# davidkelley/searchlite

Hardware: NVIDIA B200
Metric: bm25_top10_queries_per_sec (higher is better)
Workload: dtype f32

## Files before the change

### searchlite_b200/csrc/slg_engine.cu

```cuda
#include "slg_host.h"

#include <cub/cub.cuh>
#include <fcntl.h>
#include <sys/mman.h>
#include <sys/stat.h>
#include <unistd.h>

#include "slg_filter.cuh"
#include "slg_phrase.cuh"
#include "slg_postimage.cuh"
#include "slg_residency.cuh"
#include "slg_segfiles.h"

using namespace slg;

namespace slg {
std::string &open_error() {
  thread_local std::string e;
  return e;
}
cudaStream_t &pool_stream() {
  thread_local cudaStream_t s = nullptr;
  return s;
}
// ... 87 lines not shown
  d.col_stride = 0;
  d.term_ub = nullptr;
  d.term_bits = nullptr;
  d.pres_bits = nullptr;
  d.bits_stride = 0;
  d.n_terms = s->n_terms;
  d.doc_count = s->doc_count;
  d.k1p1 = s->k1 + 1.0f;
  d.min_nk = host_nk(s->min_doc_len, s->avgdl, s->k1, s->b);
  d.term_field = n_fields > 1 ? s->term_field.as<uint8_t>() : nullptr;
  for (uint32_t f = 0; f < kMaxFields; f++)
    d.min_nk_f[f] = f < n_fields ? host_nk(s->f_min_len[f], s->f_avgdl[f], s->k1, s->b) : d.min_nk;

  if (ix->resident_scores && s->n_blocks) {
    SLG_CUDA(ix, s->post_score.alloc(s->n_post_padded * 4));
    SLG_CUDA(ix, cudaMemsetAsync(s->post_score.p, 0, s->n_post_padded * 4, st));
    SLG_CUDA(ix, s->mb_max.alloc((s->n_post_padded / 32 + 1) * 4));
    SLG_CUDA(ix, cudaMemsetAsync(s->mb_max.p, 0, (s->n_post_padded / 32 + 1) * 4, st));
    slg_score_postings_kernel<<<s->n_blocks, 128, 0, st>>>(d, s->n_blocks, s->post_score.as<float>(), s->mb_max.as<float>());
    count_launch(ix);
    SLG_CUDA(ix, cudaGetLastError());
    d.post_score = s->post_score.as<float>();
    d.mb_max = s->mb_max.as<float>();
    if (ix->dense_den && s->doc_count) {
      const uint64_t stride = align_up((uint64_t)s->doc_count, 4096) + 4096;
      std::vector<uint32_t> cand;
      for (uint64_t t = 0; t < s->n_terms; t++) {
        const uint64_t df = s->h_df[t];
        if (df >= ix->dense_min_df && df * ix->dense_den >= s->doc_count) cand.push_back((uint32_t)t);
      }
      std::sort(cand.begin(), cand.end(), [&](uint32_t a, uint32_t b2) { return s->h_df[a] != s->h_df[b2] ? s->h_df[a] > s->h_df[b2] : a < b2; });
      const uint64_t max_cols = std::min<uint64_t>(65535, ix->max_column_bytes / (stride * 4));
      if (cand.size() > max_cols) cand.resize(max_cols);
      if (!cand.empty()) {
        std::vector<int32_t> tcol(s->n_terms, -1);
        for (size_t c = 0; c < cand.size(); c++) tcol[cand[c]] = (int32_t)c;
        DevBuf d_terms;
        SLG_CUDA(ix, d_terms.alloc(cand.size() * 4));
        SLG_CUDA(ix, cudaMemcpyAsync(d_terms.p, cand.data(), cand.size() * 4, cudaMemcpyHostToDevice, st));
        SLG_CUDA(ix, s->term_col.alloc(s->n_terms * 4));
        SLG_CUDA(ix, cudaMemcpyAsync(s->term_col.p, tcol.data(), s->n_terms * 4, cudaMemcpyHostToDevice, st));
        SLG_CUDA(ix, s->cols.alloc(cand.size() * stride * 4));
        SLG_CUDA(ix, cudaMemsetAsync(s->cols.p, 0, cand.size() * stride * 4, st));
        s->n_cols = (uint32_t)cand.size();
        s->col_stride = stride;
        d.col_stride = stride;
        for (size_t c0 = 0; c0 < cand.size(); c0 += 32768) {
          const uint32_t nc = (uint32_t)std::min<size_t>(32768, cand.size() - c0);
          slg_fill_columns_kernel<<<dim3(256, nc), 256, 0, st>>>(d, d_terms.as<uint32_t>() + c0, nc,
                                                                  s->cols.as<float>() + c0 * stride);
          count_launch(ix);
        }
        SLG_CUDA(ix, cudaGetLastError());
        s->tmax_stride = (uint32_t)(stride / 512);
        SLG_CUDA(ix, s->col_tmax.alloc(cand.size() * s->tmax_stride * 4));
        {
          const uint64_t warps = (uint64_t)cand.size() * s->tmax_stride;
          slg_column_tmax_kernel<<<(unsigned)((warps * 32 + 255) / 256), 256, 0, st>>>(s->cols.as<float>(), stride, (uint32_t)cand.size(),
                                                                                     s->tmax_stride, s->col_tmax.as<float>());
          count_launch(ix);
        }
        SLG_CUDA(ix, cudaGetLastError());
        SLG_CUDA(ix, cudaStreamSynchronize(st));
        s->h_term_col = std::move(tcol);
        d.cols = s->cols.as<float>();
        d.term_col = s->term_col.as<int32_t>();
        d.col_tmax = s->col_tmax.as<float>();
        d.tmax_stride = s->tmax_stride;
      }
    }
  }
  if (d.post_score && s->n_terms) {
    SLG_CUDA(ix, s->term_ub.alloc(s->n_terms * 4));
    SLG_CUDA(ix, cudaMemsetAsync(s->term_ub.p, 0, s->n_terms * 4, st));
    ScanDev sc{};
    sc.ut_term = nullptr;
    sc.ut_max = s->term_ub.as<float>();
    slg_term_max_kernel<<<dim3((unsigned)((s->n_terms + 7) / 8), kMaxSlices), 256, 0, st>>>(d, sc, (uint32_t)s->n_terms);
    count_launch(ix);
    SLG_CUDA(ix, cudaGetLastError());
    d.term_ub = s->term_ub.as<float>();
  }
  if (ix->resident_scores && ix->bitmap_den && s->doc_count && s->n_blocks) {
    const uint32_t stride = (uint32_t)align_up(((uint64_t)s->doc_count + 31) / 32, 32);
    std::vector<uint32_t> cand;
    for (uint64_t t = 0; t < s->n_terms; t++) {
      const uint64_t df = s->h_df[t];
      if (df >= 64 && df * ix->bitmap_den >= s->doc_count && (s->h_term_col.empty() || s->h_term_col[t] < 0)) cand.push_back((uint32_t)t);
    }
    std::sort(cand.begin(), cand.end(), [&](uint32_t a, uint32_t b2) { return s->h_df[a] != s->h_df[b2] ? s->h_df[a] > s->h_df[b2] : a < b2; });
    const uint64_t max_rows = std::min<uint64_t>(32768, ix->max_bitmap_bytes / ((uint64_t)stride * 4));
    if (cand.size() > max_rows) cand.resize(max_rows);
    if (!cand.empty()) {
      std::vector<int32_t> tb(s->n_terms, -1);
      for (size_t r = 0; r < cand.size(); r++) tb[cand[r]] = (int32_t)r;
      DevBuf d_terms;
      SLG_CUDA(ix, d_terms.alloc(cand.size() * 4));
      SLG_CUDA(ix, cudaMemcpyAsync(d_terms.p, cand.data(), cand.size() * 4, cudaMemcpyHostToDevice, st));
      SLG_CUDA(ix, s->term_bits.alloc(s->n_terms * 4));
      SLG_CUDA(ix, cudaMemcpyAsync(s->term_bits.p, tb.data(), s->n_terms * 4, cudaMemcpyHostToDevice, st));
      SLG_CUDA(ix, s->pres_bits.alloc(cand.size() * (uint64_t)stride * 4));
      SLG_CUDA(ix, cudaMemsetAsync(s->pres_bits.p, 0, cand.size() * (uint64_t)stride * 4, st));
      slg_fill_presence_kernel<<<dim3(64, (unsigned)cand.size()), 256, 0, st>>>(d, d_terms.as<uint32_t>(), (uint32_t)cand.size(), s->pres_bits.as<uint32_t>(), stride);
      count_launch(ix);
      SLG_CUDA(ix, cudaGetLastError());
      SLG_CUDA(ix, cudaStreamSynchronize(st));
      s->n_bitmaps = (uint32_t)cand.size();
      d.term_bits = s->term_bits.as<int32_t>();
      d.pres_bits = s->pres_bits.as<uint32_t>();
      d.bits_stride = stride;
    }
  }
  ix->ctr.resident_bytes += s->resident();
  for (auto &old : ix->segs)
    if (old->ord == s->ord) {
      ix->ctr.resident_bytes -= old->resident();
      old = std::move(seg);
      return SLG_OK;
    }
  ix->segs.push_back(std::move(seg));
  std::sort(ix->segs.begin(), ix->segs.end(), [](const auto &a, const auto &b2) { return a->ord < b2->ord; });
  return SLG_OK;
}

int32_t build_layout(slg_index *ix, Segment *s) {
  cudaStream_t st = ix->stream;
  std::vector<uint64_t> start(s->n_terms + 1);
  std::vector<uint32_t> blk(s->n_terms + 1);
  uint64_t pos = 0, nb = 0, np = 0;
  for (uint64_t t = 0; t < s->n_terms; t++) {
    start[t] = pos;
    blk[t] = (uint32_t)nb;
    uint32_t df = s->h_df[t];
    np += df;
    pos += align_up(df, kTermAlign);
    nb += (df + kBlock - 1) / kBlock;
    if (nb > 0xFFFFFFF0ull) return fail(ix, SLG_ERR_UNSUPPORTED, "segment has too many posting blocks");
  }
  start[s->n_terms] = pos;
  blk[s->n_terms] = (uint32_t)nb;
  s->n_postings = np;
  s->n_post_padded = pos + 1024;
  s->n_blocks = (uint32_t)nb;
  SLG_CUDA(ix, s->term_start.alloc((s->n_terms + 1) * 8));
  SLG_CUDA(ix, s->term_blk.alloc((s->n_terms + 1) * 4));
  SLG_CUDA(ix, s->term_df.alloc(std::max<uint64_t>(s->n_terms, 1) * 4));
  SLG_CUDA(ix, cudaMemcpyAsync(s->term_start.p, start.data(), (s->n_terms + 1) * 8, cudaMemcpyHostToDevice, st));
  SLG_CUDA(ix, cudaMemcpyAsync(s->term_blk.p, blk.data(), (s->n_terms + 1) * 4, cudaMemcpyHostToDevice, st));
  if (s->n_terms) SLG_CUDA(ix, cudaMemcpyAsync(s->term_df.p, s->h_df.data(), s->n_terms * 4, cudaMemcpyHostToDevice, st));
  SLG_CUDA(ix, s->post_doc.alloc(s->n_post_padded * 4));
  SLG_CUDA(ix, s->post_tf.alloc(s->n_post_padded));
  SLG_CUDA(ix, cudaMemsetAsync(s->post_doc.p, 0xFF, s->n_post_padded * 4, st));
  SLG_CUDA(ix, cudaMemsetAsync(s->post_tf.p, 0, s->n_post_padded, st));
  SLG_CUDA(ix, s->blk_max_doc.alloc((size_t)std::max(s->n_blocks, 1u) * 4));
  SLG_CUDA(ix, s->blk_max_tf.alloc((size_t)std::max(s->n_blocks, 1u) * 4));
  SLG_CUDA(ix, s->term_max_tf.alloc(std::max<uint64_t>(s->n_terms, 1) * 4));
  SLG_CUDA(ix, s->term_wide.alloc(std::max<uint64_t>(s->n_terms, 1) * 8));
  SLG_CUDA(ix, cudaMemsetAsync(s->term_wide.p, 0xFF, std::max<uint64_t>(s->n_terms, 1) * 8, st));
  SLG_CUDA(ix, cudaStreamSynchronize(st));
  s->h_start = std::move(start);
  return SLG_OK;
}

int32_t build_wide(slg_index *ix, Segment *s, const uint64_t *d_csr_off, const uint32_t *d_csr_tfs, const uint4 *d_ovf = nullptr,
                   uint32_t n_ovf = 0) {
  cudaStream_t st = ix->stream;
  if (!s->n_terms) return SLG_OK;
  if (s->n_blocks) {
    DevBuf bad;
    SLG_CUDA(ix, bad.alloc(4));
    SLG_CUDA(ix, cudaMemsetAsync(bad.p, 0, 4, st));
    slg_validate_postings_kernel<<<s->n_blocks, 128, 0, st>>>(s->term_start.as<uint64_t>(), s->term_blk.as<uint32_t>(), s->term_df.as<uint32_t>(),
                                                              s->n_terms, s->n_blocks, s->post_doc.as<uint32_t>(), s->doc_count, bad.as<uint32_t>());
    count_launch(ix);
    uint32_t n_bad = 0;
    SLG_CUDA(ix, cudaMemcpyAsync(&n_bad, bad.p, 4, cudaMemcpyDeviceToHost, st));
    SLG_CUDA(ix, cudaStreamSynchronize(st));
    if (n_bad)
      return fail(ix, SLG_ERR_INVALID, "segment %u: %u postings name a doc outside the segment's %u docs or break the ascending order of their list",
                  s->ord, n_bad, s->doc_count);
  }
  slg_term_max_tf_kernel<<<(unsigned)((s->n_terms + 255) / 256), 256, 0, st>>>(s->term_blk.as<uint32_t>(), s->blk_max_tf.as<float>(),
                                                                              s->n_terms, s->term_max_tf.as<float>());
  count_launch(ix);
  std::vector<float> mtf(s->n_terms);
  SLG_CUDA(ix, cudaMemcpyAsync(mtf.data(), s->term_max_tf.p, s->n_terms * 4, cudaMemcpyDeviceToHost, st));
  SLG_CUDA(ix, cudaStreamSynchronize(st));
  std::vector<uint32_t> wide_terms;
  std::vector<uint64_t> wide_off;
// ... 1421 lines not shown
```

### searchlite_b200/csrc/slg_residency.cuh

```cuda
#pragma once
#include "slg_kernels.cuh"

namespace slg {

static __global__ void __launch_bounds__(256) slg_plan_walk_kernel(SegmentDev seg, const uint32_t *ut_term, const uint32_t *row_u,
                                                              uint32_t n_rows, uint32_t tile_docs, uint32_t n_tiles,
                                                              bool column_rows, uint32_t *rng) {
  const uint32_t r = blockIdx.x;
  if (r >= n_rows) return;
  const uint32_t term = ut_term[row_u ? row_u[r] : r];
  uint32_t *out = rng + (uint64_t)r * (n_tiles + 1);
  const uint32_t step = gridDim.y * blockDim.x;
  const uint32_t first = blockIdx.y * blockDim.x + threadIdx.x;
  if (term >= seg.n_terms) {
    for (uint32_t j = first; j <= n_tiles; j += step) out[j] = 0u;
    return;
  }
  if (!column_rows && seg.term_col && seg.term_col[term] >= 0) return;
  const uint32_t df = seg.term_df[term];
  const uint32_t *d = seg.post_doc + seg.term_start[term];
  if ((uint64_t)df <= 8ull * (n_tiles + 1)) {
    for (uint32_t i = first; i <= df; i += step) {
      const uint32_t a = i ? d[i - 1] / tile_docs + 1 : 0u;
      const uint32_t b = i < df ? d[i] / tile_docs : n_tiles;
      for (uint32_t j = a; j <= b; j++) out[j] = i;
    }
  } else {
    for (uint32_t j = first; j <= n_tiles; j += step) {
      const uint64_t target = (uint64_t)j * tile_docs;
      uint32_t lo = 0, hi = df;
      while (lo < hi) {
        const uint32_t mid = (lo + hi) >> 1;
        if (d[mid] < target) lo = mid + 1;
        else hi = mid;
      }
      out[j] = lo;
    }
  }
}

static __global__ void __launch_bounds__(128) slg_score_postings_kernel(SegmentDev seg, uint32_t n_blocks, float *post_score, float *mb_max) {
  const uint32_t blk = blockIdx.x;
  if (blk >= n_blocks) return;
  __shared__ uint32_t s_term;
  if (threadIdx.x == 0) {
    uint64_t lo = 0, hi = seg.n_terms;
    while (lo + 1 < hi) {
      const uint64_t mid = (lo + hi) >> 1;
      if (seg.term_blk[mid] <= blk) lo = mid;
      else hi = mid;
    }
    s_term = (uint32_t)lo;
  }
  __syncthreads();
  const uint32_t term = s_term;
  const uint32_t i = (blk - seg.term_blk[term]) * kBlock + threadIdx.x;
  const uint32_t df = seg.term_df[term];
  const uint64_t base = seg.term_start[term];
  float s = 0.0f;
  if (i < df) {
    const uint32_t doc = seg.post_doc[base + i];
    uint32_t tf = seg.post_tf[base + i];
    const uint64_t wide = seg.term_wide[term];
    if (tf == 255u && wide != ~0ull) tf = seg.tf_wide[wide + i];
    s = bm25_contrib_fast(tf, seg.term_idf[term], seg.k1p1, seg_nk(seg, term)[doc], 1.0f);
    post_score[base + i] = s;
  }
  float m = s;
  for (int o = 16; o > 0; o >>= 1) m = fmaxf(m, __shfl_xor_sync(0xFFFFFFFFu, m, o));
  const uint32_t i0 = (blk - seg.term_blk[term]) * kBlock + (threadIdx.x & ~31u);
  if ((threadIdx.x & 31) == 0 && i0 < ((df + 31u) & ~31u)) mb_max[(base + i0) >> 5] = m;
}

static __global__ void slg_fill_columns_kernel(SegmentDev seg, const uint32_t *col_terms, uint32_t n_cols, float *cols) {
  const uint32_t c = blockIdx.y;
  if (c >= n_cols) return;
  const uint32_t term = col_terms[c];
  const uint32_t df = seg.term_df[term];
  const uint64_t base = seg.term_start[term];
  float *col = cols + (uint64_t)c * seg.col_stride;
  for (uint32_t i = blockIdx.x * blockDim.x + threadIdx.x; i < df; i += gridDim.x * blockDim.x)
    col[seg.post_doc[base + i]] = seg.post_score[base + i];
}

static __global__ void slg_fill_presence_kernel(SegmentDev seg, const uint32_t *bm_terms, uint32_t n_rows, uint32_t *bits, uint32_t stride) {
  const uint32_t r = blockIdx.y;
  if (r >= n_rows) return;
  const uint32_t term = bm_terms[r];
  const uint32_t df = seg.term_df[term];
  const uint32_t *d = seg.post_doc + seg.term_start[term];
  uint32_t *row = bits + (uint64_t)r * stride;
  for (uint32_t i = blockIdx.x * blockDim.x + threadIdx.x; i < df; i += gridDim.x * blockDim.x) {
    const uint32_t doc = d[i];
    atomicOr(row + (doc >> 5), 1u << (doc & 31));
  }
}

static __global__ void slg_column_tmax_kernel(const float *cols, uint64_t col_stride, uint32_t n_cols, uint32_t tmax_stride, float *tmax) {
  const uint64_t w = ((uint64_t)blockIdx.x * blockDim.x + threadIdx.x) >> 5;
  const int lane = threadIdx.x & 31;
  if (w >= (uint64_t)n_cols * tmax_stride) return;
  const uint32_t c = (uint32_t)(w / tmax_stride), j = (uint32_t)(w % tmax_stride);
  const float4 *p = reinterpret_cast<const float4 *>(cols + (uint64_t)c * col_stride + (uint64_t)j * 512) + lane;
  float m = 0.0f;
#pragma unroll
  for (int i = 0; i < 4; i++) {
    const float4 v = p[i * 32];
    m = fmaxf(m, fmaxf(fmaxf(v.x, v.y), fmaxf(v.z, v.w)));
  }
  for (int o = 16; o > 0; o >>= 1) m = fmaxf(m, __shfl_xor_sync(0xFFFFFFFFu, m, o));
  if (lane == 0) tmax[w] = m;
}

}
```

### searchlite_b200/csrc/slg_scan_kernel.cuh

```cuda
#pragma once
#include "slg_stream_kernel.cuh"

namespace slg {

constexpr uint32_t kScanChunk = 4096;
constexpr int kScanWarps = 8;
constexpr uint32_t kScanQueue = 512;

struct __align__(16) ScanPair {
  uint64_t base;
  uint32_t df;
  uint32_t qslot_t;
  uint32_t qi;
  float w;
  float others;
  float ne_prefix;
  int32_t filter;
  uint32_t first_item;
  uint32_t pad[2];
};

struct ScanDev {
  const uint32_t *ut_term;
  float *ut_max;
// ... 205 lines not shown

static __global__ void __launch_bounds__(1024) slg_scan_order_kernel(WarpBatchDev wb, ScanDev sc) {
  __shared__ uint32_t s_hist[33], s_cur[33], s_carry;
  const uint32_t tid = threadIdx.x, nthr = blockDim.x;
  const uint32_t n = wb.n_queries * kWarpMaxTerms;
  if (tid < 33) s_hist[tid] = 0u;
  __syncthreads();
  for (uint32_t i = tid; i < n; i += nthr) {
    const uint32_t df = sc.pairs[i].df;
    if (df) atomicAdd(&s_hist[32 - __clz(df)], 1u);
  }
  __syncthreads();
  if (tid == 0) {
    uint32_t run = 0;
    for (int b = 0; b < 33; b++) {
      s_cur[b] = run;
      run += s_hist[b];
    }
    *sc.n_pairs = run;
    s_carry = 0;
  }
  __syncthreads();
  for (uint32_t i = tid; i < n; i += nthr) {
    const uint32_t df = sc.pairs[i].df;
    if (df) sc.order[atomicAdd(&s_cur[32 - __clz(df)], 1u)] = i;
  }
  __syncthreads();
  const uint32_t np = *sc.n_pairs;
  __shared__ uint32_t s_scan[1024];
  for (uint32_t b0 = 0; b0 < np; b0 += nthr) {
    const uint32_t i = b0 + tid;
    uint32_t c = 0;
    if (i < np) c = (sc.pairs[sc.order[i]].df + sc.chunk - 1) / sc.chunk;
    s_scan[tid] = c;
    __syncthreads();
    for (uint32_t o = 1; o < nthr; o <<= 1) {
      const uint32_t v = tid >= o ? s_scan[tid - o] : 0u;
      __syncthreads();
      s_scan[tid] += v;
      __syncthreads();
    }
    const uint32_t excl = s_scan[tid] - c + s_carry;
    if (i < np) {
      sc.item_start[i] = excl;
      sc.pairs[sc.order[i]].first_item = excl;
    }
    __syncthreads();
    if (tid == nthr - 1) s_carry += s_scan[tid];
    __syncthreads();
  }
  if (tid == 0) {
    sc.item_start[np] = s_carry;
    *sc.n_items = min(s_carry, sc.items_cap);
  }
}

static __global__ void __launch_bounds__(256) slg_scan_items_kernel(ScanDev sc) {
  const uint32_t i = blockIdx.x * blockDim.x + threadIdx.x;
  const uint32_t n_items = *sc.n_items, np = *sc.n_pairs;
  if (i >= n_items) return;
  uint32_t lo = 0, hi = np;
  while (lo + 1 < hi) {
    const uint32_t mid = (lo + hi) >> 1;
    if (sc.item_start[mid] <= i) lo = mid;
    else hi = mid;
  }
  sc.items[i] = lo;
}

template <bool PRUNE, bool POOLS, bool MUST>
__global__ void __launch_bounds__(kScanWarps * 32, 4) slg_scan_kernel(SegmentDev seg, WarpBatchDev wb, ScanDev sc) {
  __shared__ __align__(16) unsigned long long s_cand[kScanWarps][kWarpCand];
  __shared__ uint32_t s_hist[kScanWarps][POOLS ? 256 : 1];
  __shared__ uint32_t s_qidx[kScanWarps][kScanQueue];
  __shared__ float s_qval[kScanWarps][kScanQueue];
  const int lane = threadIdx.x & 31, warp = threadIdx.x >> 5;
  unsigned long long *cand = s_cand[warp];
  uint32_t *q_idx = s_qidx[warp];
  float *q_val = s_qval[warp];
  const uint32_t k = wb.k;
  const uint32_t n_all = *sc.n_items;
  const uint32_t item_lo = (uint32_t)(((uint64_t)n_all * sc.part_lo) >> 8), n_items = (uint32_t)(((uint64_t)n_all * sc.part_hi) >> 8);
  uint32_t *work = sc.counter + (sc.part_lo ? 1 : 0);
  const float inv_docs = 1.0f / (float)max(seg.doc_count, 1u);
  unsigned long long n_scanned = 0, n_verified = 0, n_lookups = 0;
  uint32_t n_dropped = 0, n_done = 0;
  WarpCand wc;

  uint32_t item = 0;
  if (lane == 0) item = item_lo + atomicAdd(work, 1u);
  item = __shfl_sync(0xFFFFFFFFu, item, 0);
  while (item < n_items) {
    uint32_t next_item = 0;
    if (lane == 0) next_item = item_lo + atomicAdd(work, 1u);
    const uint32_t pi = __ldg(sc.order + __ldg(sc.items + item));
    const ScanPair pr = sc.pairs[pi];
    const unsigned long long thr0 = load_threshold(wb, pr.qi);
    const uint32_t chunk = item - pr.first_item;
    const bool have_thr0 = thr0 != kThrInit;
    const float thr0_score = __uint_as_float((uint32_t)(thr0 >> 32));
    if (PRUNE && have_thr0 && pr.ne_prefix * 1.00002f < thr0_score) {
      n_dropped++;
    } else {
      n_done++;
      wc.begin(cand, thr0, k, lane, 0u, POOLS ? s_hist[warp] : nullptr);
      const uint32_t qslot = pr.qslot_t >> 3, t = pr.qslot_t & 7u;
      const QTerm *qts = wb.qterms + (uint64_t)qslot * kWarpMaxTerms;
      const uint32_t nt = __ldg(&wb.qheads[qslot].nt);
      uint64_t m_base = 0;
      uint64_t m_col = 0;
      uint64_t m_bits = 0;
      uint32_t m_df = 0, m_kind = 0;
      float m_w = 0.0f, m_ub = 0.0f, m_dens = 0.0f;
      if (lane < (int)nt) {
        const QTerm q = qts[lane];
        if (q.flags & 1u) {
          m_w = q.weight;
          m_ub = __fmul_rn(sc.ut_max[q.uterm], q.weight);
          if (q.flags & 4u) {
            m_kind = 2;
            if (MUST) {
              m_col = q.sc_base;
              m_base = q.base;
            } else {
              m_base = q.sc_base;
            }
          } else if (q.term < seg.n_terms) {
            m_kind = 1;
            m_base = q.base;
            m_df = __ldg(seg.term_df + q.term);
            m_dens = (float)m_df * inv_docs;
            m_bits = ~0ull;
            if (seg.term_bits) {
              const int32_t row = __ldg(seg.term_bits + q.term);
              if (row >= 0) m_bits = (uint64_t)row * seg.bits_stride;
            }
          }
        }
      }
      const float my_ub = __shfl_sync(0xFFFFFFFFu, m_ub, t);
      const float4 *sp = reinterpret_cast<const float4 *>(wb.scores + pr.base);
      const uint32_t i0 = chunk * sc.chunk, i1 = min(pr.df, i0 + sc.chunk);
      n_scanned += i1 - i0;
      uint32_t cut = 0u;
      auto recut = [&]() {
        cut = 0u;
        if (wc.thr != kThrInit) {
          const float cf = __uint_as_float((uint32_t)(wc.thr >> 32)) * 0.99998f - pr.others * 1.00002f;
          cut = cf > 0.0f ? __float_as_uint(cf) : 0u;
        }
      };
      recut();
      uint32_t nq = 0, qhead = 0;
      auto verify_round = [&](uint32_t n) {
        bool alive = lane < (int)n;
        uint32_t doc = 0u;
        float v = 0.0f;
        if (alive) {
          doc = q_idx[(qhead + lane) & (kScanQueue - 1u)];
          v = q_val[(qhead + lane) & (kScanQueue - 1u)];
        }
        qhead += n;
        nq -= n;
        alive = alive && __float_as_uint(v) >= cut;
        n_verified += alive ? 1u : 0u;
        if (alive && pr.filter >= 0) alive = (__ldg(wb.filter_bits[pr.filter] + (doc >> 5)) >> (doc & 31)) & 1u;
        const bool must = MUST;
        const float thr_s = wc.thr == kThrInit ? 0.0f : __uint_as_float((uint32_t)(wc.thr >> 32)) * 0.99998f;
        float c[kWarpMaxTerms];
        float known = v, unknown = pr.others;
#pragma unroll
        for (int u = 0; u < (int)kWarpMaxTerms; u++) {
          c[u] = 0.0f;
          const uint32_t kind = __shfl_sync(0xFFFFFFFFu, m_kind, u);
          if (kind != 2u || u == (int)t) continue;
          const uint64_t cb = __shfl_sync(0xFFFFFFFFu, MUST ? m_col : m_base, u);
          const float w = __shfl_sync(0xFFFFFFFFu, m_w, u), ub = __shfl_sync(0xFFFFFFFFu, m_ub, u);
          if (alive) {
            c[u] = __fmul_rn(__ldg(seg.cols + cb + doc), w);
            known += c[u];
            unknown -= ub;
            if (must && c[u] == 0.0f) alive = false;
          }
        }
        alive = alive && (known + fmaxf(unknown, 0.0f)) * 1.0001f >= thr_s;
        bool stand_back = false;
        const int n_rounds = sc.two_rounds ? 2 : 1;
#pragma unroll 1
        for (int round = 0; round < n_rounds; round++)
#pragma unroll
        for (int u = 0; u < (int)kWarpMaxTerms; u++) {
          const uint32_t kind = __shfl_sync(0xFFFFFFFFu, m_kind, u);
          if (kind != 1u || u == (int)t) continue;
          const float ub = __shfl_sync(0xFFFFFFFFu, m_ub, u);
          const bool higher = !must && (ub > my_ub || (ub == my_ub && u < (int)t));
          if (n_rounds == 2 && higher != (round == 1)) continue;
          if (!__any_sync(0xFFFFFFFFu, alive)) break;
          const uint64_t pb = __shfl_sync(0xFFFFFFFFu, m_base, u), bo = __shfl_sync(0xFFFFFFFFu, m_bits, u);
          const uint32_t dfu = __shfl_sync(0xFFFFFFFFu, m_df, u);
          const float w = __shfl_sync(0xFFFFFFFFu, m_w, u), dens = __shfl_sync(0xFFFFFFFFu, m_dens, u);
          if (alive) {
            n_lookups++;
            const uint32_t *dp = seg.post_doc + pb;
            bool held = true;
            if (bo != ~0ull) held = (__ldg(seg.pres_bits + bo + (doc >> 5)) >> (doc & 31)) & 1u;
            const uint32_t at = held ? lower_bound_interp(dp, dfu, doc, dens) : dfu;
            if (at < dfu && __ldg(dp + at) == doc) {
              if (higher) stand_back = true;
              c[u] = __fmul_rn(__ldg(wb.scores + pb + at), w);
              known += c[u];
            } else if (must) {
              stand_back = true;
            }
            if (!higher) unknown -= ub;
            alive = !stand_back && (known + fmaxf(unknown, 0.0f)) * 1.0001f >= thr_s;
          }
        }
        if (__any_sync(0xFFFFFFFFu, alive)) {
          float sx = 0.0f;
#pragma unroll
          for (int u = 0; u < (int)kWarpMaxTerms; u++) {
            const float cu = u == (int)t ? v : c[u];
            if (cu != 0.0f) sx = __fadd_rn(sx, cu);
          }
          wc.offer(seg, wb, pr.qi, pr.filter, alive, doc, sx);
          recut();
        }
        __syncwarp();
      };
#pragma unroll 1
      for (uint32_t b = i0; b < i1; b += 256) {
        const uint32_t ia = b + lane * 4, ib = ia + 128;
        float4 va = make_float4(0, 0, 0, 0), vb = make_float4(0, 0, 0, 0);
        if (ia < i1) va = __ldg(sp + (ia >> 2));
        if (ib < i1) vb = __ldg(sp + (ib >> 2));
        float x[8] = {va.x, va.y, va.z, va.w, vb.x, vb.y, vb.z, vb.w};
        uint32_t todo = 0u;
#pragma unroll
        for (int e = 0; e < 8; e++) {
          x[e] = __fmul_rn(x[e], pr.w);
          const uint32_t idx = (e < 4 ? ia : ib) + (e & 3);
          if (__float_as_uint(x[e]) >= cut && x[e] != 0.0f && idx < i1) todo |= 1u << e;
        }
        if (!__any_sync(0xFFFFFFFFu, todo != 0u)) continue;
        const uint4 *dp4 = reinterpret_cast<const uint4 *>(seg.post_doc + pr.base);
        uint4 da = make_uint4(0, 0, 0, 0), db = make_uint4(0, 0, 0, 0);
        if (todo & 0x0Fu) da = __ldg(dp4 + (ia >> 2));
        if (todo & 0xF0u) db = __ldg(dp4 + (ib >> 2));
        const uint32_t dd[8] = {da.x, da.y, da.z, da.w, db.x, db.y, db.z, db.w};
        {
          const uint32_t mine = __popc(todo);
          uint32_t incl = mine;
#pragma unroll
          for (int o = 1; o < 32; o <<= 1) {
            const uint32_t nb = __shfl_up_sync(0xFFFFFFFFu, incl, o);
            if (lane >= o) incl += nb;
          }
          uint32_t at = qhead + nq + incl - mine;
#pragma unroll
          for (int e = 0; e < 8; e++)
            if ((todo >> e) & 1u) {
              q_idx[at & (kScanQueue - 1u)] = dd[e];
              q_val[at & (kScanQueue - 1u)] = x[e];
              at++;
            }
          nq += __shfl_sync(0xFFFFFFFFu, incl, 31);
          __syncwarp();
        }
        while (nq >= 32u) verify_round(32u);
      }
      while (nq) verify_round(min(nq, 32u));
      wc.merge(wb, pr.qi);
    }
    item = __shfl_sync(0xFFFFFFFFu, next_item, 0);
  }
  if (sc.counters) {
#pragma unroll
    for (int o = 16; o > 0; o >>= 1) {
      n_verified += __shfl_xor_sync(0xFFFFFFFFu, n_verified, o);
      n_lookups += __shfl_xor_sync(0xFFFFFFFFu, n_lookups, o);
    }
    if (lane == 0) {
      if (n_scanned) atomicAdd(sc.counters + 0, n_scanned);
      if (n_verified) atomicAdd(sc.counters + 4, n_verified);
      if (n_dropped) atomicAdd(sc.counters + 5, (unsigned long long)n_dropped);
      if (n_lookups) atomicAdd(sc.counters + 6, n_lookups);
      if (n_done) atomicAdd(sc.counters + 3, (unsigned long long)n_done);
    }
  }
}

}
```

### searchlite_b200/csrc/slg_search.cu

```cuda
#include "slg_host.h"
#include "slg_residency.cuh"

using namespace slg;

namespace {

struct TermSet {
  std::vector<uint32_t> key, val;
  uint32_t mask = 0;
  explicit TermSet(size_t expect) {
    size_t n = 64;
    while (n < expect * 2) n <<= 1;
    key.assign(n, 0xFFFFFFFFu);
    val.assign(n, 0);
    mask = (uint32_t)n - 1;
  }
  uint32_t get(uint32_t term, std::vector<uint32_t> &ut) {
    uint32_t h = (term * 0x9E3779B1u) & mask;
    for (;;) {
      if (key[h] == term) return val[h];
      if (key[h] == 0xFFFFFFFFu) {
        key[h] = term;
        val[h] = (uint32_t)ut.size();
        ut.push_back(term);
// ... 774 lines not shown
  SLG_CUDA(ix, cudaSetDevice(ix->device));
  slg_import_thresholds_kernel<<<(bt->Q + 255) / 256, 256, 0, ix->stream>>>(bt->thr_key, static_cast<const unsigned long long *>(dev_keys), bt->Q);
  count_launch(ix);
  SLG_CUDA(ix, cudaGetLastError());
  return SLG_OK;
}

int32_t slg_batch_run_sweep(slg_batch_t *bt, int32_t sync) {
  if (!bt) return SLG_ERR_INVALID;
  slg_index *ix = bt->ix;
  if (!bt->seeds_done) return fail(ix, SLG_ERR_INVALID, "slg_batch_run_sweep follows slg_batch_run_seeds");
  SLG_CUDA(ix, cudaSetDevice(ix->device));
  int32_t rc = run_batch(bt, false, true);
  if (rc) return rc;
  bt->seeds_done = false;
  return sync ? finish_timing(bt) : SLG_OK;
}

int32_t slg_batch_set_threshold_board(slg_batch_t *bt, void *local_board, void *const *peer_boards, uint32_t n_peers, uint32_t epoch) {
  if (!bt) return SLG_ERR_INVALID;
  slg_index *ix = bt->ix;
  if (!local_board) {
    bt->board = nullptr;
    bt->n_board_peers = 0;
    return SLG_OK;
  }
  if (n_peers > kMaxBoardPeers || (n_peers && !peer_boards)) return fail(ix, SLG_ERR_INVALID, "a threshold board has at most %u peers", kMaxBoardPeers);
  if (epoch == 0) return fail(ix, SLG_ERR_INVALID, "board epochs start at 1 and rise with every batch");
  if (ix->segs.size() != 1) return fail(ix, SLG_ERR_UNSUPPORTED, "the threshold board needs one segment per handle (shard == segment)");
  bt->board = static_cast<unsigned long long *>(local_board);
  for (uint32_t p = 0; p < kMaxBoardPeers; p++) bt->peer_board[p] = p < n_peers ? static_cast<unsigned long long *>(peer_boards[p]) : nullptr;
  bt->n_board_peers = n_peers;
  bt->board_epoch = epoch;
  return SLG_OK;
}

int32_t slg_batch_enable_stats(slg_batch_t *bt, int32_t on) {
  if (!bt) return SLG_ERR_INVALID;
  bt->want_stats = on != 0;
  return SLG_OK;
}

static unsigned char *result_block(slg_batch *bt) {
  return bt->results + (bt->n_segs_run > 1 ? (size_t)bt->n_segs_run * bt->result_stride : 0);
}

int32_t slg_batch_device_results(slg_batch_t *bt, void **dev_hits, void **dev_counts) {
  if (!bt || !dev_hits || !dev_counts) return SLG_ERR_INVALID;
  unsigned char *r = result_block(bt);
  *dev_hits = r;
  *dev_counts = r + (size_t)bt->Q * bt->k * sizeof(HitDev);
  return SLG_OK;
}

int32_t slg_batch_packed_results(slg_batch_t *bt, void **dev_block, uint64_t *n_bytes) {
  if (!bt || !dev_block || !n_bytes) return SLG_ERR_INVALID;
  *dev_block = result_block(bt);
  *n_bytes = (uint64_t)bt->Q * bt->k * sizeof(HitDev) + (uint64_t)bt->Q * 4 + (bt->reranked ? (uint64_t)bt->Q * bt->k * 4 : 0);
  return SLG_OK;
}

int32_t slg_batch_fetch(slg_batch_t *bt, slg_hit_t *out_hits, uint32_t *out_counts, slg_stats_t *out_stats) {
  if (!bt || !out_hits || !out_counts) return SLG_ERR_INVALID;
  slg_index *ix = bt->ix;
  SLG_CUDA(ix, cudaSetDevice(ix->device));
  cudaStream_t st = ix->stream;
  static_assert(sizeof(slg_hit_t) == sizeof(HitDev), "hit layout");
  const size_t hb = (size_t)bt->Q * bt->k * sizeof(slg_hit_t), cb = (size_t)bt->Q * 4, sb = (size_t)bt->Q * 40 + 64;
  unsigned char *pin = static_cast<unsigned char *>(bt->pinned) + bt->pinned_result_off;
  SLG_CUDA(ix, cudaMemcpyAsync(pin, result_block(bt), hb + cb, cudaMemcpyDeviceToHost, st));
  SLG_CUDA(ix, cudaMemcpyAsync(pin + bt->result_stride, bt->stats, sb, cudaMemcpyDeviceToHost, st));
  SLG_CUDA(ix, cudaStreamSynchronize(st));
  ix->ctr.last_d2h_bytes = hb + cb + sb;
  std::memcpy(out_hits, pin, hb);
  std::memcpy(out_counts, pin + hb, cb);
  const unsigned long long *sv = reinterpret_cast<const unsigned long long *>(pin + bt->result_stride);
  const unsigned long long *ic = sv + (size_t)bt->Q * 5;
  ix->ctr.last_postings_scattered = ic[0];
  ix->ctr.last_subtiles_skipped = ic[1];
  ix->ctr.last_column_blocks_streamed = ic[2];
  ix->ctr.last_items = ic[3];
  ix->ctr.last_postings_verified = ic[4];
  ix->ctr.last_items_dropped = ic[5];
  if (out_stats) {
    for (uint32_t q = 0; q < bt->Q; q++) {
      out_stats[q].scored_docs = sv[q * 4 + 0];
      out_stats[q].postings_advanced = sv[q * 4 + 1];
      out_stats[q].blocks_skipped = sv[q * 4 + 2];
      out_stats[q].candidates_examined = sv[q * 4 + 3];
      out_stats[q].total_matches = sv[(size_t)bt->Q * 4 + q];
    }
  }
  return SLG_OK;
}

int32_t slg_batch_copy_results_device(slg_batch_t *bt, void *dst_hits, void *dst_counts) {
  if (!bt || !dst_hits || !dst_counts) return SLG_ERR_INVALID;
  slg_index *ix = bt->ix;
  SLG_CUDA(ix, cudaSetDevice(ix->device));
  void *dh, *dc;
  slg_batch_device_results(bt, &dh, &dc);
  SLG_CUDA(ix, cudaMemcpyAsync(dst_hits, dh, (size_t)bt->Q * bt->k * sizeof(HitDev), cudaMemcpyDeviceToDevice, ix->stream));
  SLG_CUDA(ix, cudaMemcpyAsync(dst_counts, dc, (size_t)bt->Q * 4, cudaMemcpyDeviceToDevice, ix->stream));
  return SLG_OK;
}

int32_t slg_batch_cursor_seen(slg_batch_t *bt, uint8_t *out_seen) {
  if (!bt || !out_seen) return SLG_ERR_INVALID;
  slg_index *ix = bt->ix;
  SLG_CUDA(ix, cudaSetDevice(ix->device));
  for (uint32_t q = 0; q < bt->Q; q++) out_seen[q] = 1;
  if (!bt->has_cursor) return SLG_OK;
  std::vector<uint32_t> saw(bt->Q);
  SLG_CUDA(ix, cudaMemcpyAsync(saw.data(), bt->cursor_saw, (size_t)bt->Q * 4, cudaMemcpyDeviceToHost, ix->stream));
  SLG_CUDA(ix, cudaStreamSynchronize(ix->stream));
  for (uint32_t q = 0; q < bt->Q; q++)
    if (bt->h_has_cursor[q]) out_seen[q] = saw[q] ? 1 : 0;
  return SLG_OK;
}

int32_t slg_batch_free(slg_batch_t *bt) {
  if (!bt) return SLG_OK;
  cudaSetDevice(bt->ix->device);
  {
    PoolScope pool_scope(bt->ix->stream);
    delete bt;
  }
  return SLG_OK;
}

int32_t slg_search_batch(slg_index_t *ix, const slg_query_t *queries, uint32_t n_queries, uint32_t k, slg_exec_t exec,
                         uint32_t bmw_block_size, slg_hit_t *out_hits, uint32_t *out_counts, slg_stats_t *out_stats) {
  if (!ix) return SLG_ERR_INVALID;
  if (!out_hits || !out_counts) return fail(ix, SLG_ERR_INVALID, "output buffers are NULL");
  slg_batch_t *bt = nullptr;
  int32_t rc = slg_batch_prepare(ix, queries, n_queries, k, exec, bmw_block_size, &bt);
  if (rc) return rc;
  bt->want_stats = out_stats != nullptr;
  rc = slg_batch_run(bt, 0);
  if (rc == SLG_OK) rc = slg_batch_fetch(bt, out_hits, out_counts, out_stats);
  if (rc == SLG_OK && ix->segs.size() == 1 && bt->U) {
    float ms = 0;
    if (cudaEventElapsedTime(&ms, ix->ev[2], ix->ev[3]) == cudaSuccess) {
      ix->ctr.score_ms_total += ms;
      ix->ctr.last_score_ms = ms;
    }
    if (cudaEventElapsedTime(&ms, ix->ev[0], ix->ev[1]) == cudaSuccess) ix->ctr.last_batch_ms = ms;
  }
  slg_batch_free(bt);
  return rc;
}

static int32_t merge_packed(slg_index_t *ix, const void *dev_gathered, uint64_t shard_stride, uint32_t n_shards, uint32_t n_queries, uint32_t k,
                            slg_hit_t *out_hits, uint32_t *out_counts, bool hybrid, float *out_vs) {
  if (!ix || !dev_gathered || !out_hits || !out_counts || !n_shards || !n_queries || !k) return SLG_ERR_INVALID;
  SLG_CUDA(ix, cudaSetDevice(ix->device));
  cudaStream_t st = ix->stream;
  const size_t hb = (size_t)n_queries * k * sizeof(HitDev), cb = (size_t)n_queries * 4, vb = hybrid ? (size_t)n_queries * k * 4 : 0;
  if (shard_stride == 0) shard_stride = hb + cb + vb;
  if (shard_stride % 4 || shard_stride < hb + cb + vb)
    return fail(ix, SLG_ERR_INVALID, "shard stride %llu does not hold %zu bytes", (unsigned long long)shard_stride, hb + cb + vb);
  size_t msmem = (size_t)n_shards * k * sizeof(HitDev);
  if (msmem > ix->smem_optin || n_shards > kMaxMergeLists) return fail(ix, SLG_ERR_UNSUPPORTED, "merge of %u shards x k=%u does not fit shared memory", n_shards, k);
  PoolScope pool_scope(st);
  DevBuf ob;
  SLG_CUDA(ix, ob.alloc(hb + cb + vb));
// ... 55 lines not shown
```

### searchlite_b200/csrc/slg_stream_kernel.cuh

```cuda
#pragma once
#include "slg_async.cuh"
#include "slg_items_kernel.cuh"

namespace slg {

constexpr uint32_t kColBlock = 256;
constexpr int kSparseWarps = 4;
constexpr int kColWarps = 16;
constexpr uint32_t kColMaxSlots = 4096;

struct __align__(16) ColQ {
  uint32_t qslot, qi;
  int32_t filter;
  uint8_t nsp, ncol, unit_w, off;
  uint16_t slot[8];
  float extra;
  uint32_t pad[3];
};

struct StreamDev {
  ColQ *colq;
  uint32_t *n_colq;
  uint32_t *ucol;
  uint32_t *n_ucol;
  uint32_t *col_slot;
  uint32_t *sparse_counter, *col_counter;
  uint32_t stage_cap;
  uint32_t col_resident;
  uint32_t n_smax;
  uint32_t strict;
  unsigned long long *counters;
};

__device__ __forceinline__ bool colq_prune(const WarpBatchDev &wb, const float *ut_max, uint32_t qslot, uint32_t qi, uint32_t nt, float &extra) {
  const unsigned long long thr = load_threshold(wb, qi);
  float ub[kWarpMaxTerms];
  bool col[kWarpMaxTerms];
  for (uint32_t t = 0; t < kWarpMaxTerms; t++) {
    ub[t] = 0.0f;
    col[t] = false;
    if (t < nt) {
      const QTerm &q = wb.qterms[(uint64_t)qslot * kWarpMaxTerms + t];
      if (q.flags & 1u) ub[t] = __fmul_rn(ut_max[q.uterm], q.weight);
      col[t] = (q.flags & 5u) == 5u;
    }
  }
  extra = 0.0f;
  bool any_essential_col = false;
  for (uint32_t t = 0; t < nt; t++) {
    float pre = 0.0f;
    for (uint32_t u = 0; u < nt; u++)
      if (ub[u] < ub[t] || (ub[u] == ub[t] && u >= t)) pre += ub[u];
    const bool ne = thr != kThrInit && pre * 1.00002f < __uint_as_float((uint32_t)(thr >> 32));
    if (col[t]) any_essential_col = any_essential_col || !ne;
    else if (ne) extra += ub[t];
  }
  return any_essential_col;
}

static __global__ void __launch_bounds__(1024) slg_colgroups_kernel(SegmentDev seg, WarpBatchDev wb, StreamDev sd, uint32_t n_cols, const float *ut_max) {
  const uint32_t tid = threadIdx.x, nthr = blockDim.x;
  for (uint32_t c = tid; c < n_cols; c += nthr) sd.col_slot[c] = 0u;
  if (tid == 0) {
    *sd.n_colq = 0u;
    *sd.n_ucol = 0u;
  }
  __syncthreads();
  for (uint32_t slot = tid; slot < wb.n_queries; slot += nthr) {
    const QHead h = wb.qheads[slot];
    float extra;
    if (ut_max && !colq_prune(wb, ut_max, slot, h.qi, h.nt, extra)) continue;
    for (uint32_t t = 0; t < h.nt; t++) {
      const QTerm &q = wb.qterms[(uint64_t)slot * kWarpMaxTerms + t];
      if ((q.flags & 5u) == 5u) sd.col_slot[q.term] = 1u;
    }
  }
  __syncthreads();
  {
    __shared__ uint32_t s_scan[1024];
    __shared__ uint32_t s_carry;
    if (tid == 0) s_carry = 0u;
    __syncthreads();
    for (uint32_t base = 0; base < n_cols; base += nthr) {
      const uint32_t c = base + tid;
      const uint32_t flag = c < n_cols && sd.col_slot[c] ? 1u : 0u;
// ... 667 lines not shown
        const uint32_t span_tot = __shfl_sync(0xFFFFFFFFu, tot, nspan - 1);
        if (span_tot == 0) {
          j0 = j1;
          continue;
        }
        __syncwarp();
        if (lane == 0) mbar_arrive_expect_tx(bar, span_tot * 8u);
        __syncwarp();
#pragma unroll
        for (int h = 0; h < 2; h++) {
          const uint32_t e = lane + 32 * h, t = e & 7, j = e >> 3;
          if (len[h] && j >= j0 && j < j1) {
            const uint32_t off = cum[e] - base;
            bulk_copy_g2s(sdoc + off, seg.post_doc + qt[t].base + alo[h], len[h] * 4u, bar);
            bulk_copy_g2s(ssc + off, wb.scores + qt[t].base + alo[h], len[h] * 4u, bar);
          }
        }
        mbar_wait(bar, parity);
        parity ^= 1u;
        for (uint32_t j = j0; j < j1; j++) {
          if (sd.strict)
            sparse_sub<true>(seg, wb, head, qt, rb + j, cum + j * 8, base, nsp, colmask, unit_w, rest[j], (sub0 + j) * sub_docs, sub_docs, own, sdoc, ssc,
                             pend, wc, lane);
          else
            sparse_sub_bounded(seg, wb, head, qt, cum + j * 8, base, nsp, colmask, unit_w, wmx, rest[j], (sub0 + j) * sub_docs, sub_docs, sdoc, ssc, cmx,
                               wc, lane);
        }
        j0 = j1;
      }
      wc.merge(wb, head.qi);
    }
    if (n_post > 0x40000000u) {
      n_post_total += n_post;
      n_post = 0;
    }
    item = __shfl_sync(0xFFFFFFFFu, next_item, 0);
  }
  if (sd.counters) {
    n_post_total += n_post;
#pragma unroll
    for (int o = 16; o > 0; o >>= 1) n_post_total += __shfl_xor_sync(0xFFFFFFFFu, n_post_total, o);
    if (lane == 0) {
      if (n_post_total) atomicAdd(sd.counters + 0, n_post_total);
      if (n_items) atomicAdd(sd.counters + 3, (unsigned long long)n_items);
    }
  }
}

__device__ __forceinline__ uint32_t lower_bound_interp(const uint32_t *dp, uint32_t n, uint32_t doc, float dens) {
  uint32_t lo = 0, hi = n;
  float est = (float)doc * dens;
#pragma unroll 1
  for (int it = 0; it < 4 && lo < hi; it++) {
    const uint32_t pos = min(max(est < 0.0f ? 0u : (uint32_t)est, lo), hi - 1u);
    const uint32_t d = __ldg(dp + pos);
    if (d < doc) lo = pos + 1u;
    else hi = pos;
    if (d == doc) break;
    est = (float)pos + ((float)doc - (float)d) * dens;
  }
  while (lo < hi) {
    const uint32_t mid = (lo + hi) >> 1;
    if (__ldg(dp + mid) < doc) lo = mid + 1u;
    else hi = mid;
  }
  return lo;
}

__device__ __forceinline__ float verify_doc(const SegmentDev &seg, const WarpBatchDev &wb, const QTerm *qts, uint32_t nt, bool have, uint32_t doc,
                                            uint32_t &holders) {
  float s = 0.0f;
  holders = 0u;
  if (have) {
    for (uint32_t u = 0; u < nt; u++) {
      const uint32_t flags = __ldg(&qts[u].flags);
      if (!(flags & 1u)) continue;
      float c = 0.0f;
      if (flags & 4u) {
        c = __ldg(seg.cols + __ldg(&qts[u].sc_base) + doc);
      } else {
        const uint32_t term = __ldg(&qts[u].term);
        if (term < seg.n_terms) {
          const uint64_t base = __ldg(&qts[u].base);
          const uint32_t *dp = seg.post_doc + base;
          const uint32_t end = __ldg(seg.term_df + term);
          bool held = true;
          if (seg.term_bits) {
            const int32_t row = __ldg(seg.term_bits + term);
            if (row >= 0) held = (__ldg(seg.pres_bits + (uint64_t)row * seg.bits_stride + (doc >> 5)) >> (doc & 31)) & 1u;
          }
          const uint32_t lo = held ? lower_bound_interp(dp, end, doc, (float)end / (float)max(seg.doc_count, 1u)) : end;
          if (lo < end && __ldg(dp + lo) == doc) {
            c = __ldg(wb.scores + base + lo);
            holders |= 1u << u;
          }
        }
      }
      if (c != 0.0f) s = __fadd_rn(s, __fmul_rn(c, __ldg(&qts[u].weight)));
    }
  }
  return s;
}

__host__ __device__ inline size_t column_smem(uint32_t resident, uint32_t n_smax) {
  return (size_t)2 * resident * kColBlock * 4 + (((size_t)n_smax * 4 + 15) & ~(size_t)15) + (size_t)kColWarps * kWarpCand * 8 + 16;
}

template <bool PRUNE, bool POOLS>
__global__ void __launch_bounds__(kColWarps * 32) slg_score_columns_kernel(SegmentDev seg, WarpBatchDev wb, StreamDev sd) {
  extern __shared__ __align__(16) unsigned char smem_raw[];
  __shared__ uint32_t s_hist[kColWarps][POOLS ? 256 : 1];
  const int tid = threadIdx.x, lane = tid & 31, warp = tid >> 5;
  const uint32_t n_used = *sd.n_ucol, n_colq = *sd.n_colq;
  const uint32_t resident = min(sd.col_resident, n_used), n_smax = min(n_used, sd.n_smax);
  float *buf = reinterpret_cast<float *>(smem_raw);
  float *smax = buf + (size_t)2 * sd.col_resident * kColBlock;
  unsigned long long *cand = reinterpret_cast<unsigned long long *>(reinterpret_cast<unsigned char *>(smax) + (((size_t)sd.n_smax * 4 + 15) & ~(size_t)15)) +
                             (size_t)warp * kWarpCand;
  unsigned long long *bar = reinterpret_cast<unsigned long long *>(smem_raw + column_smem(sd.col_resident, sd.n_smax) - 16);
  const uint32_t k = wb.k;
  const uint32_t n_blocks = (seg.doc_count + kColBlock - 1) / kColBlock;
  if (n_colq == 0 || n_used == 0) return;
  if (tid == 0) {
    mbar_init(bar, 1);
    mbar_init(bar + 1, 1);
    asm volatile("fence.mbarrier_init.release.cluster;" ::: "memory");
  }
  asm volatile("fence.proxy.async.shared::cta;" ::: "memory");
  __syncthreads();
  unsigned long long n_tests = 0, n_looked = 0;
  WarpCand wc;
  auto fetch = [&](uint32_t blk, uint32_t b) {
    if (warp == 0) {
      if (lane == 0) mbar_arrive_expect_tx(bar + b, resident * kColBlock * 4u);
      __syncwarp();
      for (uint32_t s = lane; s < resident; s += 32)
        bulk_copy_g2s(buf + ((size_t)b * sd.col_resident + s) * kColBlock, seg.cols + (uint64_t)sd.ucol[s] * seg.col_stride + (uint64_t)blk * kColBlock,
                      kColBlock * 4u, bar + b);
    }
  };
  uint32_t parity[2] = {0u, 0u};
  uint32_t blk = blockIdx.x;
  if (blk < n_blocks) fetch(blk, 0);
  uint32_t b = 0;
  for (; blk < n_blocks; blk += gridDim.x, b ^= 1u) {
    const uint32_t nxt = blk + gridDim.x;
    if (nxt < n_blocks) fetch(nxt, b ^ 1u);
    mbar_wait(bar + b, parity[b]);
    parity[b] ^= 1u;
    const float *cb = buf + (size_t)b * sd.col_resident * kColBlock;
    const uint32_t d0 = blk * kColBlock;
    for (uint32_t s = warp; s < n_smax; s += kColWarps) {
      const float4 *p = s < resident ? reinterpret_cast<const float4 *>(cb + (size_t)s * kColBlock)
                                     : reinterpret_cast<const float4 *>(seg.cols + (uint64_t)sd.ucol[s] * seg.col_stride + d0);
      uint32_t top = 0u;
#pragma unroll
      for (uint32_t x = 0; x < kColBlock / 128; x++) {
        const float4 v = p[x * 32 + lane];
        top = max(top, max(max(__float_as_uint(v.x), __float_as_uint(v.y)), max(__float_as_uint(v.z), __float_as_uint(v.w))));
      }
      top = __reduce_max_sync(0xFFFFFFFFu, top);
      if (lane == 0) smax[s] = __uint_as_float(top);
    }
    __syncthreads();
    for (uint32_t c0 = warp * 32; c0 < n_colq; c0 += kColWarps * 32) {
      ColQ cq;
      cq.ncol = 0;
      unsigned long long thr = ~0ull;
      const bool live = c0 + lane < n_colq;
      if (live) {
        cq = sd.colq[c0 + lane];
        thr = load_threshold(wb, cq.qi);
      }
      bool look = false;
      if (live && !cq.off) {
        n_tests++;
// ... 130 lines not shown
```

Measured before the change: 520,800.

## Replace bitmap-guarded binary search with rank-indexed presence bitmaps for posting lookups

```diff
diff --git a/searchlite_b200/csrc/slg_engine.cu b/searchlite_b200/csrc/slg_engine.cu
--- a/searchlite_b200/csrc/slg_engine.cu
+++ b/searchlite_b200/csrc/slg_engine.cu
@@ -193,7 +193,7 @@
     d.term_ub = s->term_ub.as<float>();
   }
   if (ix->resident_scores && ix->bitmap_den && s->doc_count && s->n_blocks) {
-    const uint32_t stride = (uint32_t)align_up(((uint64_t)s->doc_count + 31) / 32, 32);
+    const uint32_t stride = presence_row_words(s->doc_count);
     std::vector<uint32_t> cand;
     for (uint64_t t = 0; t < s->n_terms; t++) {
       const uint64_t df = s->h_df[t];
@@ -215,7 +215,18 @@
       slg_fill_presence_kernel<<<dim3(64, (unsigned)cand.size()), 256, 0, st>>>(d, d_terms.as<uint32_t>(), (uint32_t)cand.size(), s->pres_bits.as<uint32_t>(), stride);
       count_launch(ix);
       SLG_CUDA(ix, cudaGetLastError());
+      DevBuf d_totals;
+      SLG_CUDA(ix, d_totals.alloc(cand.size() * 4));
+      slg_presence_rank_kernel<<<(unsigned)cand.size(), kRankThreads, 0, st>>>(s->pres_bits.as<uint32_t>(), stride, (uint32_t)cand.size(), d_totals.as<uint32_t>());
+      count_launch(ix);
+      SLG_CUDA(ix, cudaGetLastError());
+      std::vector<uint32_t> totals(cand.size());
+      SLG_CUDA(ix, cudaMemcpyAsync(totals.data(), d_totals.p, cand.size() * 4, cudaMemcpyDeviceToHost, st));
       SLG_CUDA(ix, cudaStreamSynchronize(st));
+      for (size_t r = 0; r < cand.size(); r++)
+        if (totals[r] != s->h_df[cand[r]])
+          return fail(ix, SLG_ERR_INVALID, "segment %u: presence bitmap of term %u counts %u docs, its list holds %u", s->ord, cand[r], totals[r],
+                      s->h_df[cand[r]]);
       s->n_bitmaps = (uint32_t)cand.size();
       d.term_bits = s->term_bits.as<int32_t>();
       d.pres_bits = s->pres_bits.as<uint32_t>();
diff --git a/searchlite_b200/csrc/slg_residency.cuh b/searchlite_b200/csrc/slg_residency.cuh
--- a/searchlite_b200/csrc/slg_residency.cuh
+++ b/searchlite_b200/csrc/slg_residency.cuh
@@ -83,6 +83,29 @@
     col[seg.post_doc[base + i]] = seg.post_score[base + i];
 }
 
+constexpr uint32_t kPresUnitDocs = 224;
+constexpr uint32_t kPresUnitWords = 8;
+
+__host__ __device__ inline uint32_t presence_row_words(uint32_t doc_count) {
+  return (doc_count + kPresUnitDocs - 1) / kPresUnitDocs * kPresUnitWords;
+}
+
+__device__ __forceinline__ bool presence_lookup(const SegmentDev &seg, uint64_t row_off, uint32_t doc, uint32_t &at) {
+  const uint32_t u = doc / kPresUnitDocs, r = doc - u * kPresUnitDocs;
+  const uint4 *p = reinterpret_cast<const uint4 *>(seg.pres_bits + row_off + (uint64_t)u * kPresUnitWords);
+  const uint4 a = __ldg(p), b = __ldg(p + 1);
+  const uint32_t w[kPresUnitWords] = {a.x, a.y, a.z, a.w, b.x, b.y, b.z, b.w};
+  const uint32_t wi = 1u + (r >> 5), bit = r & 31u;
+  uint32_t word = 0u, n = w[0];
+#pragma unroll
+  for (uint32_t i = 1; i < kPresUnitWords; i++) {
+    if (i < wi) n += __popc(w[i]);
+    if (i == wi) word = w[i];
+  }
+  at = n + __popc(word & ((1u << bit) - 1u));
+  return (word >> bit) & 1u;
+}
+
 static __global__ void slg_fill_presence_kernel(SegmentDev seg, const uint32_t *bm_terms, uint32_t n_rows, uint32_t *bits, uint32_t stride) {
   const uint32_t r = blockIdx.y;
   if (r >= n_rows) return;
@@ -92,8 +115,52 @@
   uint32_t *row = bits + (uint64_t)r * stride;
   for (uint32_t i = blockIdx.x * blockDim.x + threadIdx.x; i < df; i += gridDim.x * blockDim.x) {
     const uint32_t doc = d[i];
-    atomicOr(row + (doc >> 5), 1u << (doc & 31));
+    const uint32_t u = doc / kPresUnitDocs, rem = doc - u * kPresUnitDocs;
+    atomicOr(row + (uint64_t)u * kPresUnitWords + 1u + (rem >> 5), 1u << (rem & 31));
   }
+}
+
+constexpr uint32_t kRankThreads = 1024;
+static __global__ void __launch_bounds__(kRankThreads) slg_presence_rank_kernel(uint32_t *bits, uint32_t stride, uint32_t n_rows, uint32_t *totals) {
+  __shared__ uint32_t s_warp[kRankThreads / 32 + 1];
+  const uint32_t r = blockIdx.x;
+  if (r >= n_rows) return;
+  const int lane = threadIdx.x & 31, warp = threadIdx.x >> 5;
+  uint32_t *row = bits + (uint64_t)r * stride;
+  const uint32_t n_units = stride / kPresUnitWords;
+  uint32_t carry = 0u;
+  for (uint32_t u0 = 0; u0 < n_units; u0 += kRankThreads) {
+    const uint32_t u = u0 + threadIdx.x;
+    uint32_t c = 0u;
+    if (u < n_units) {
+      const uint4 *p = reinterpret_cast<const uint4 *>(row + (uint64_t)u * kPresUnitWords);
+      const uint4 a = p[0], b = p[1];
+      c = __popc(a.y) + __popc(a.z) + __popc(a.w) + __popc(b.x) + __popc(b.y) + __popc(b.z) + __popc(b.w);
+    }
+    uint32_t incl = c;
+#pragma unroll
+    for (int o = 1; o < 32; o <<= 1) {
+      const uint32_t v = __shfl_up_sync(0xFFFFFFFFu, incl, o);
+      if (lane >= o) incl += v;
+    }
+    if (lane == 31) s_warp[warp] = incl;
+    __syncthreads();
+    if (warp == 0) {
+      uint32_t t = s_warp[lane], ti = t;
+#pragma unroll
+      for (int o = 1; o < 32; o <<= 1) {
+        const uint32_t v = __shfl_up_sync(0xFFFFFFFFu, ti, o);
+        if (lane >= o) ti += v;
+      }
+      s_warp[lane] = ti - t;
+      if (lane == 31) s_warp[kRankThreads / 32] = ti;
+    }
+    __syncthreads();
+    if (u < n_units) row[(uint64_t)u * kPresUnitWords] = carry + s_warp[warp] + incl - c;
+    carry += s_warp[kRankThreads / 32];
+    __syncthreads();
+  }
+  if (threadIdx.x == 0) totals[r] = carry;
 }
 
 static __global__ void slg_column_tmax_kernel(const float *cols, uint64_t col_stride, uint32_t n_cols, uint32_t tmax_stride, float *tmax) {
diff --git a/searchlite_b200/csrc/slg_scan_kernel.cuh b/searchlite_b200/csrc/slg_scan_kernel.cuh
--- a/searchlite_b200/csrc/slg_scan_kernel.cuh
+++ b/searchlite_b200/csrc/slg_scan_kernel.cuh
@@ -311,8 +311,8 @@
   const uint32_t n_all = *sc.n_items;
   const uint32_t item_lo = (uint32_t)(((uint64_t)n_all * sc.part_lo) >> 8), n_items = (uint32_t)(((uint64_t)n_all * sc.part_hi) >> 8);
   uint32_t *work = sc.counter + (sc.part_lo ? 1 : 0);
-  const float inv_docs = 1.0f / (float)max(seg.doc_count, 1u);
-  unsigned long long n_scanned = 0, n_verified = 0, n_lookups = 0;
+  unsigned long long n_scanned = 0;
+  uint32_t n_lane_verified = 0, n_lane_bit_lookups = 0, n_lane_searches = 0;
   uint32_t n_dropped = 0, n_done = 0;
   WarpCand wc;
 
@@ -338,9 +338,8 @@
       const uint32_t nt = __ldg(&wb.qheads[qslot].nt);
       uint64_t m_base = 0;
       uint64_t m_col = 0;
-      uint64_t m_bits = 0;
       uint32_t m_df = 0, m_kind = 0;
-      float m_w = 0.0f, m_ub = 0.0f, m_dens = 0.0f;
+      float m_w = 0.0f, m_ub = 0.0f;
       if (lane < (int)nt) {
         const QTerm q = qts[lane];
         if (q.flags & 1u) {
@@ -358,11 +357,10 @@
             m_kind = 1;
             m_base = q.base;
             m_df = __ldg(seg.term_df + q.term);
-            m_dens = (float)m_df * inv_docs;
-            m_bits = ~0ull;
-            if (seg.term_bits) {
-              const int32_t row = __ldg(seg.term_bits + q.term);
-              if (row >= 0) m_bits = (uint64_t)row * seg.bits_stride;
+            const int32_t row = seg.term_bits ? __ldg(seg.term_bits + q.term) : -1;
+            if (row >= 0) {
+              m_kind = 3;
+              m_df = (uint32_t)row;
             }
           }
         }
@@ -392,7 +390,7 @@
         qhead += n;
         nq -= n;
         alive = alive && __float_as_uint(v) >= cut;
-        n_verified += alive ? 1u : 0u;
+        n_lane_verified += alive ? 1u : 0u;
         if (alive && pr.filter >= 0) alive = (__ldg(wb.filter_bits[pr.filter] + (doc >> 5)) >> (doc & 31)) & 1u;
         const bool must = MUST;
         const float thr_s = wc.thr == kThrInit ? 0.0f : __uint_as_float((uint32_t)(wc.thr >> 32)) * 0.99998f;
@@ -420,24 +418,33 @@
 #pragma unroll
         for (int u = 0; u < (int)kWarpMaxTerms; u++) {
           const uint32_t kind = __shfl_sync(0xFFFFFFFFu, m_kind, u);
-          if (kind != 1u || u == (int)t) continue;
+          if (!(kind & 1u) || u == (int)t) continue;
           const float ub = __shfl_sync(0xFFFFFFFFu, m_ub, u);
           const bool higher = !must && (ub > my_ub || (ub == my_ub && u < (int)t));
           if (n_rounds == 2 && higher != (round == 1)) continue;
           if (!__any_sync(0xFFFFFFFFu, alive)) break;
-          const uint64_t pb = __shfl_sync(0xFFFFFFFFu, m_base, u), bo = __shfl_sync(0xFFFFFFFFu, m_bits, u);
+          const uint64_t pb = __shfl_sync(0xFFFFFFFFu, m_base, u);
           const uint32_t dfu = __shfl_sync(0xFFFFFFFFu, m_df, u);
-          const float w = __shfl_sync(0xFFFFFFFFu, m_w, u), dens = __shfl_sync(0xFFFFFFFFu, m_dens, u);
+          const float w = __shfl_sync(0xFFFFFFFFu, m_w, u);
           if (alive) {
-            n_lookups++;
-            const uint32_t *dp = seg.post_doc + pb;
-            bool held = true;
-            if (bo != ~0ull) held = (__ldg(seg.pres_bits + bo + (doc >> 5)) >> (doc & 31)) & 1u;
-            const uint32_t at = held ? lower_bound_interp(dp, dfu, doc, dens) : dfu;
-            if (at < dfu && __ldg(dp + at) == doc) {
-              if (higher) stand_back = true;
-              c[u] = __fmul_rn(__ldg(wb.scores + pb + at), w);
-              known += c[u];
+            bool held;
+            uint32_t at = 0u;
+            if (kind == 3u) {
+              n_lane_bit_lookups++;
+              held = presence_lookup(seg, (uint64_t)dfu * seg.bits_stride, doc, at);
+            } else {
+              n_lane_searches++;
+              const uint32_t *dp = seg.post_doc + pb;
+              at = lower_bound_interp(dp, dfu, doc, (float)dfu * (1.0f / (float)max(seg.doc_count, 1u)));
+              held = at < dfu && __ldg(dp + at) == doc;
+            }
+            if (held) {
+              if (higher) {
+                stand_back = true;
+              } else {
+                c[u] = __fmul_rn(__ldg(wb.scores + pb + at), w);
+                known += c[u];
+              }
             } else if (must) {
               stand_back = true;
             }
@@ -504,16 +511,19 @@
     item = __shfl_sync(0xFFFFFFFFu, next_item, 0);
   }
   if (sc.counters) {
+    unsigned long long n_verified = n_lane_verified, n_bit_lookups = n_lane_bit_lookups, n_searches = n_lane_searches;
 #pragma unroll
     for (int o = 16; o > 0; o >>= 1) {
       n_verified += __shfl_xor_sync(0xFFFFFFFFu, n_verified, o);
-      n_lookups += __shfl_xor_sync(0xFFFFFFFFu, n_lookups, o);
+      n_bit_lookups += __shfl_xor_sync(0xFFFFFFFFu, n_bit_lookups, o);
+      n_searches += __shfl_xor_sync(0xFFFFFFFFu, n_searches, o);
     }
     if (lane == 0) {
       if (n_scanned) atomicAdd(sc.counters + 0, n_scanned);
       if (n_verified) atomicAdd(sc.counters + 4, n_verified);
       if (n_dropped) atomicAdd(sc.counters + 5, (unsigned long long)n_dropped);
-      if (n_lookups) atomicAdd(sc.counters + 6, n_lookups);
+      if (n_bit_lookups) atomicAdd(sc.counters + 6, n_bit_lookups);
+      if (n_searches) atomicAdd(sc.counters + 7, n_searches);
       if (n_done) atomicAdd(sc.counters + 3, (unsigned long long)n_done);
     }
   }
diff --git a/searchlite_b200/csrc/slg_search.cu b/searchlite_b200/csrc/slg_search.cu
--- a/searchlite_b200/csrc/slg_search.cu
+++ b/searchlite_b200/csrc/slg_search.cu
@@ -880,6 +880,8 @@
   ix->ctr.last_items = ic[3];
   ix->ctr.last_postings_verified = ic[4];
   ix->ctr.last_items_dropped = ic[5];
+  if (getenv("SLG_SCAN_TRACE"))
+    fprintf(stderr, "[slg scan] verified %llu, sparse look-ups answered by a presence bitmap %llu, by lower_bound_interp %llu\n", ic[4], ic[6], ic[7]);
   if (out_stats) {
     for (uint32_t q = 0; q < bt->Q; q++) {
       out_stats[q].scored_docs = sv[q * 4 + 0];
diff --git a/searchlite_b200/csrc/slg_stream_kernel.cuh b/searchlite_b200/csrc/slg_stream_kernel.cuh
--- a/searchlite_b200/csrc/slg_stream_kernel.cuh
+++ b/searchlite_b200/csrc/slg_stream_kernel.cuh
@@ -1,6 +1,7 @@
 #pragma once
 #include "slg_async.cuh"
 #include "slg_items_kernel.cuh"
+#include "slg_residency.cuh"
 
 namespace slg {
 
@@ -834,16 +835,19 @@
         const uint32_t term = __ldg(&qts[u].term);
         if (term < seg.n_terms) {
           const uint64_t base = __ldg(&qts[u].base);
-          const uint32_t *dp = seg.post_doc + base;
-          const uint32_t end = __ldg(seg.term_df + term);
-          bool held = true;
-          if (seg.term_bits) {
-            const int32_t row = __ldg(seg.term_bits + term);
-            if (row >= 0) held = (__ldg(seg.pres_bits + (uint64_t)row * seg.bits_stride + (doc >> 5)) >> (doc & 31)) & 1u;
-          }
-          const uint32_t lo = held ? lower_bound_interp(dp, end, doc, (float)end / (float)max(seg.doc_count, 1u)) : end;
-          if (lo < end && __ldg(dp + lo) == doc) {
-            c = __ldg(wb.scores + base + lo);
+          const int32_t row = seg.term_bits ? __ldg(seg.term_bits + term) : -1;
+          bool held;
+          uint32_t at = 0u;
+          if (row >= 0) {
+            held = presence_lookup(seg, (uint64_t)row * seg.bits_stride, doc, at);
+          } else {
+            const uint32_t *dp = seg.post_doc + base;
+            const uint32_t end = __ldg(seg.term_df + term);
+            at = lower_bound_interp(dp, end, doc, (float)end / (float)max(seg.doc_count, 1u));
+            held = at < end && __ldg(dp + at) == doc;
+          }
+          if (held) {
+            c = __ldg(wb.scores + base + at);
             holders |= 1u << u;
           }
         }
```

Result: faster. 590,300 (median of 6 runs) (+13.4%).
